# toposware/certificate-stark

Measured on NVIDIA B200. Metric: state_transition_prove_throughput, higher is better.
Workload: dtype u64 (f63 modular)

## Files before the change

certificate_stark_b200/csrc/prover.cu:

```cuda
#include "prover_ctx.cuh"

extern "C" {

csg_ctx *csg_create(int device) {
    int count = 0;
    if (cudaGetDeviceCount(&count) != cudaSuccess || device < 0 || device >= count) return nullptr;
    if (cudaSetDevice(device) != cudaSuccess) return nullptr;
    csg_ctx *ctx = new csg_ctx();
    ctx->device = device;
    if (cudaStreamCreateWithFlags(&ctx->st.s, cudaStreamNonBlocking) != cudaSuccess) { delete ctx; return nullptr; }
    return ctx;
}
void csg_destroy(csg_ctx *ctx) {
    if (!ctx) return;
    cudaSetDevice(ctx->device);
    cudaStreamSynchronize(ctx->st.s);
    cudaStream_t s = ctx->st.s;
    if (ctx->ev_a) { cudaEventDestroy(ctx->ev_a); cudaEventDestroy(ctx->ev_b); }
    for (auto e : ctx->cons_ev) if (e) cudaEventDestroy(e);
    for (auto e : ctx->chunk_ev) cudaEventDestroy(e);
    for (auto &e : ctx->comm_ev) { cudaEventDestroy(e.first); cudaEventDestroy(e.second); }
    if (ctx->ev_intt) { cudaEventDestroy(ctx->ev_intt); cudaEventDestroy(ctx->ev_gathered); }
    if (ctx->comm_stream.s) { cudaStreamSynchronize(ctx->comm_stream.s); cudaStreamDestroy(ctx->comm_stream.s); }
    ctx->comm.reset();
    if (ctx->copy_stream) cudaStreamDestroy(ctx->copy_stream);
    for (auto b : ctx->stage_buf) if (b) cudaFreeHost(b);
    for (auto e : ctx->stage_ev) if (e) cudaEventDestroy(e);
    if (ctx->h2d_a) { cudaEventDestroy(ctx->h2d_a); cudaEventDestroy(ctx->h2d_b); }
    many_delete(ctx->many);
    delete ctx;
    cudaStreamDestroy(s);
}
const char *csg_last_error(const csg_ctx *ctx) { return ctx ? ctx->err.c_str() : "no context (CUDA device unavailable)"; }
void csg_free(void *p) { free(p); }

int csg_set_air(csg_ctx *ctx, int air_id, size_t trace_len, const csg_options *opt, const uint64_t *pub, size_t npub) {
    return guarded(ctx, [&] { ctx->set_air(air_id, trace_len, opt, pub, npub); });
}
int csg_load_trace(csg_ctx *ctx, const uint64_t *trace, int repr) { return guarded(ctx, [&] { if (!trace) throw ArgError("null trace"); ctx->load_trace(trace, repr); }); }
int csg_reload_resident_trace(csg_ctx *ctx) { return guarded(ctx, [&] { ctx->reload_resident(); }); }
int csg_prove_loaded(csg_ctx *ctx, uint8_t **proof, size_t *proof_len) {
    return guarded(ctx, [&] { if (!proof || !proof_len) throw ArgError("null output"); ctx->prove_loaded(proof, proof_len); });
}
int csg_prove(csg_ctx *ctx, int air_id, const uint64_t *trace, int repr, size_t trace_len, const uint64_t *pub, size_t npub, const csg_options *opt,
              uint8_t **proof, size_t *proof_len) {
    return guarded(ctx, [&] {
        if (!trace || !proof || !proof_len) throw ArgError("null argument");
        csg_ctx::check_repr(repr);
        ctx->set_air(air_id, trace_len, opt, pub, npub);
        ctx->prove_loaded(proof, proof_len, trace, repr);
    });
}
int csg_prove_trace(csg_ctx *ctx, const uint64_t *trace, int repr, uint8_t **proof, size_t *proof_len) {
    return guarded(ctx, [&] {
        if (!trace || !proof || !proof_len) throw ArgError("null argument");
        csg_ctx::check_repr(repr);
        ctx->need(S_AIR, "csg_set_air must be called first");
        ctx->prove_loaded(proof, proof_len, trace, repr);
    });
}
int csg_prefetch_trace(csg_ctx *ctx, const uint64_t *trace, int repr) { return guarded(ctx, [&] { ctx->prefetch_trace(trace, repr); }); }
int csg_prove_prefetched(csg_ctx *ctx, const uint64_t *next_trace, int next_repr, uint8_t **proof, size_t *proof_len) {
    return guarded(ctx, [&] {
        if (!proof || !proof_len) throw ArgError("null argument");
        ctx->prove_prefetched(next_trace, next_repr, proof, proof_len);
    });
}
int csg_prove_columns(csg_ctx *ctx, int air_id, const uint64_t *const *columns, int repr, size_t trace_len, const uint64_t *pub, size_t npub,
                      const csg_options *opt, uint8_t **proof, size_t *proof_len) {
    return guarded(ctx, [&] {
        if (!columns || !proof || !proof_len) throw ArgError("null argument");
        csg_ctx::check_repr(repr);
        ctx->set_air(air_id, trace_len, opt, pub, npub);
        ctx->prove_loaded(proof, proof_len, nullptr, repr, columns);
    });
}
static int prove_many(csg_ctx *ctx, int air_id, size_t count, ManyTraces traces, int repr, size_t trace_len, const uint64_t *pubs, size_t npub,
                      const csg_options *opt, uint8_t **proofs, size_t *proof_lens) {
    if (proofs && proof_lens)
        for (size_t k = 0; k < count; k++) { proofs[k] = nullptr; proof_lens[k] = 0; }
    return guarded(ctx, [&] {
        if (ctx->comm && ctx->comm->world > 1) throw std::runtime_error("csg_prove_many does not run on a context attached to a group");
        if (!ctx->many) ctx->many = many_new();
        ctx->stage_timer.discard(); ctx->query_timer.discard();
        try { many_prove(ctx->many, ctx->st, air_id, count, traces, repr, trace_len, pubs, npub, opt, proofs, proof_lens, ctx->tm); }
        catch (const ManyArgError &e) { throw ArgError(e.what()); }
    });
}
int csg_prove_many(csg_ctx *ctx, int air_id, size_t count, const uint64_t *const *traces, int repr, size_t trace_len, const uint64_t *pubs, size_t npub,
                   const csg_options *opt, uint8_t **proofs, size_t *proof_lens) {
    return prove_many(ctx, air_id, count, ManyTraces{traces, nullptr}, repr, trace_len, pubs, npub, opt, proofs, proof_lens);
}
int csg_prove_many_device(csg_ctx *ctx, int air_id, size_t count, const uint64_t *traces_dev, int repr, size_t trace_len, const uint64_t *pubs,
                          size_t npub, const csg_options *opt, uint8_t **proofs, size_t *proof_lens) {
    return prove_many(ctx, air_id, count, ManyTraces{nullptr, traces_dev}, repr, trace_len, pubs, npub, opt, proofs, proof_lens);
}
void *csg_host_alloc(size_t bytes) {
    void *p = nullptr;
    if (!bytes || cudaHostAlloc(&p, bytes, cudaHostAllocPortable) != cudaSuccess) { cudaGetLastError(); return nullptr; }
    return p;
}
void csg_host_free(void *p) { if (p) cudaFreeHost(p); }
int csg_host_register(void *p, size_t bytes) {
    if (!p || !bytes) return CSG_ERR_ARG;
    if (cudaHostRegister(p, bytes, cudaHostRegisterDefault) != cudaSuccess) { cudaGetLastError(); return CSG_ERR_CUDA; }
    return CSG_OK;
}
int csg_host_unregister(void *p) {
    if (!p) return CSG_ERR_ARG;
    if (cudaHostUnregister(p) != cudaSuccess) { cudaGetLastError(); return CSG_ERR_CUDA; }
    return CSG_OK;
}
int csg_extend_and_commit_trace(csg_ctx *ctx, uint8_t root[32]) { return guarded(ctx, [&] { ctx->extend_and_commit_trace(root); }); }
int csg_eval_constraints(csg_ctx *ctx, const uint64_t *t_coeffs, const uint64_t *b_coeffs) {
    return guarded(ctx, [&] {
        ctx->need(S_AIR, "csg_set_air must be called first");
        if (ctx->d > 1) {
            std::vector<xe> t = mont_xvec(t_coeffs, 2 * ctx->air.num_constraints(), ctx->d), bb = mont_xvec(b_coeffs, 2 * ctx->air.assertions.size(), ctx->d);
            bb.push_back(x_zero());
            ctx->eval_constraints_x(t.data(), bb.data());
            return;
        }
        std::vector<fe> t = mont_vec(t_coeffs, 2 * ctx->air.num_constraints()), bb = mont_vec(b_coeffs, 2 * ctx->air.assertions.size());
        bb.push_back(0);
        ctx->eval_constraints(t.data(), bb.data());
    });
}
int csg_commit_composition(csg_ctx *ctx, uint8_t root[32]) { return guarded(ctx, [&] { ctx->commit_composition(root); }); }
int csg_ood_ext(csg_ctx *ctx, const uint64_t *z, uint64_t *frame_cur, uint64_t *frame_next, uint64_t *comp) {
    return guarded(ctx, [&] {
        if (!z || !frame_cur || !frame_next || !comp) throw ArgError("null argument");
        const int d = ctx->d;
        if (d == 1) { csg_ctx *c = ctx; c->ood(to_mont(z[0] % P)); for (size_t i = 0; i < c->air.width; i++) { frame_cur[i] = from_mont(c->ood_cur[i]); frame_next[i] = from_mont(c->ood_next[i]); }
                      for (size_t r = 0; r < c->ce; r++) comp[r] = from_mont(c->ood_comp[r]); return; }
        ctx->ood_x(mont_xvec(z, 1, d)[0]);
        for (size_t c = 0; c < ctx->air.width; c++)
            for (int j = 0; j < d; j++) { frame_cur[c * d + j] = from_mont(ctx->xood_cur[c].c[j]); frame_next[c * d + j] = from_mont(ctx->xood_next[c].c[j]); }
        for (size_t r = 0; r < ctx->ce; r++) for (int j = 0; j < d; j++) comp[r * d + j] = from_mont(ctx->xood_comp[r].c[j]);
    });
}
int csg_ood(csg_ctx *ctx, uint64_t z, uint64_t *frame_cur, uint64_t *frame_next, uint64_t *comp) {
    return guarded(ctx, [&] {
        if (ctx->d != 1) throw ArgError("with a field extension the out-of-domain point has several words: use csg_ood_ext");
        ctx->ood(to_mont(z % P));
        for (size_t c = 0; c < ctx->air.width; c++) { frame_cur[c] = from_mont(ctx->ood_cur[c]); frame_next[c] = from_mont(ctx->ood_next[c]); }
        for (size_t r = 0; r < ctx->ce; r++) comp[r] = from_mont(ctx->ood_comp[r]);
    });
}
int csg_deep(csg_ctx *ctx, const uint64_t *trace_ab, const uint64_t *comp_d, const uint64_t lambda_mu[2]) {
    return guarded(ctx, [&] {
        ctx->need(S_AIR, "csg_set_air must be called first");
        if (ctx->d > 1) {
            std::vector<xe> ab = mont_xvec(trace_ab, 2 * ctx->air.width, ctx->d), dd = mont_xvec(comp_d, ctx->ce, ctx->d), lm = mont_xvec(lambda_mu, 2, ctx->d);
            ctx->deep_x(ab.data(), dd.data(), lm[0], lm[1]);
            return;
        }
        std::vector<fe> ab = mont_vec(trace_ab, 2 * ctx->air.width), d = mont_vec(comp_d, ctx->ce);
        ctx->deep(ab.data(), d.data(), to_mont(lambda_mu[0] % P), to_mont(lambda_mu[1] % P));
    });
}
int csg_fri_commit_layer(csg_ctx *ctx, uint8_t root[32]) { return guarded(ctx, [&] { ctx->fri_commit_layer(root); }); }
int csg_fri_fold(csg_ctx *ctx, uint64_t alpha) {
    return guarded(ctx, [&] { if (ctx->d != 1) throw ArgError("with a field extension alpha has several words: use csg_fri_fold_ext"); ctx->fri_fold(to_mont(alpha % P)); });
}
int csg_fri_fold_ext(csg_ctx *ctx, const uint64_t *alpha) {
    return guarded(ctx, [&] { if (!alpha) throw ArgError("null argument"); ctx->fri_fold_x(mont_xvec(alpha, 1, ctx->d)[0]); });
}
int csg_fri_remainder(csg_ctx *ctx, uint64_t *out, size_t cap, size_t *len) {
    return guarded(ctx, [&] {
        ctx->need(S_DEEP, "the DEEP composition must be computed first");
        const FriLayer &L = *ctx->fri[ctx->nfri - 1];
        if (cap < L.m * ctx->d) throw ArgError("remainder buffer too small");
        std::vector<uint64_t> rem = ctx->remainder();
        memcpy(out, rem.data(), rem.size() * 8);
        *len = rem.size();
    });
}
static std::vector<size_t> checked_positions(const uint64_t *positions, size_t npos, size_t nleaves) {
    if (!positions || npos == 0 || npos > 255) throw ArgError("between 1 and 255 query positions");
    std::vector<size_t> pos(positions, positions + npos);
    std::vector<size_t> sorted(pos);
    std::sort(sorted.begin(), sorted.end());
    if (sorted.back() >= nleaves) throw ArgError("query position outside the evaluation domain");
    if (std::adjacent_find(sorted.begin(), sorted.end()) != sorted.end()) throw ArgError("query positions must be distinct");
    return pos;
}
static void copy_opening(const std::vector<uint64_t> &r, const std::vector<uint8_t> &p, uint64_t *rows, uint8_t *paths, size_t cap, size_t *paths_len) {
    if (!rows || !paths || !paths_len) throw ArgError("null output");
    if (p.size() > cap) throw ArgError("path buffer too small");
    memcpy(rows, r.data(), r.size() * 8);
    memcpy(paths, p.data(), p.size());
    *paths_len = p.size();
}
int csg_open_trace(csg_ctx *ctx, const uint64_t *positions, size_t npos, uint64_t *rows, uint8_t *paths, size_t cap, size_t *paths_len) {
    return guarded(ctx, [&] {
        ctx->need(S_COMMITTED, "the trace must be committed first");
        std::vector<size_t> pos = checked_positions(positions, npos, ctx->lde_n);
        const size_t w = ctx->air.width;
        copy_opening(ctx->open_rows(ctx->d_lde.p, (unsigned)w, (unsigned)ctx->b, w * ctx->n, ctx->n, pos, true), ctx->open_paths(ctx->d_tnodes, ctx->lde_n, pos, ctx->subtrees() ? &ctx->d_ttop : nullptr), rows, paths, cap, paths_len);
    });
}
int csg_open_composition(csg_ctx *ctx, const uint64_t *positions, size_t npos, uint64_t *rows, uint8_t *paths, size_t cap, size_t *paths_len) {
    return guarded(ctx, [&] {
        ctx->need(S_COMPOSED, "the composition polynomial must be committed first");
        std::vector<size_t> pos = checked_positions(positions, npos, ctx->lde_n);
        const size_t cw = ctx->ce * ctx->d;
        copy_opening(ctx->open_rows(ctx->d_clde.p, (unsigned)cw, (unsigned)ctx->b, cw * ctx->n, ctx->n, pos, true), ctx->open_paths(ctx->d_cnodes, ctx->lde_n, pos, ctx->subtrees() ? &ctx->d_ctop : nullptr), rows, paths, cap, paths_len);
    });
}
int csg_open_fri_layer(csg_ctx *ctx, size_t layer, const uint64_t *positions, size_t npos, uint64_t *rows, uint8_t *paths, size_t cap, size_t *paths_len) {
    return guarded(ctx, [&] {
        ctx->need(S_DEEP, "the DEEP composition must be computed first");
        if (layer >= ctx->nfri || !ctx->fri[layer]->committed) throw ArgError("no such committed FRI layer");
        const FriLayer &L = *ctx->fri[layer];
        std::vector<size_t> pos = checked_positions(positions, npos, L.m / 4);
        copy_opening(ctx->open_fri_rows(L, pos), ctx->open_paths(L.nodes, L.m / 4, pos), rows, paths, cap, paths_len);
    });
}

}
```

certificate_stark_b200/csrc/prover_ctx.cuh:

```cuda
#pragma once
#include <algorithm>
#include <chrono>
#include <cstdlib>
#include <cstring>
#include <memory>
#include <string>
#include <vector>

#include "../../include/csg.h"
#include "comm.cuh"
#include "commit.cuh"
#include "constraints.cuh"
#include "ext_stages.cuh"
#include "hash.cuh"
#include "host/air_desc.hpp"
#include "host/batch_plan.hpp"
#include "host/proof_common.hpp"
#include "host/transcript.hpp"
#include "many/many.cuh"
#include "ntt.cuh"
#include "stages.cuh"
#include "witness.cuh"


namespace csg {
using namespace f63;

namespace {

struct StateError : std::runtime_error { using std::runtime_error::runtime_error; };
struct ArgError : std::runtime_error { using std::runtime_error::runtime_error; };

struct FriLayer {
    DBuf<fe> owned;
    const fe *evals = nullptr;
    size_t m = 0;
    DBuf<uint32_t> nodes;
    bool committed = false;
};

enum Stage { S_NONE, S_AIR, S_TRACE, S_COMMITTED, S_EVALUATED, S_COMPOSED, S_OOD, S_DEEP };

class Timer {
  public:
    ~Timer() { for (auto &p : own_) { cudaEventDestroy(p.first); cudaEventDestroy(p.second); } }
    void start(Stream &st) {
        if (crowded()) flush();
        if (used_ == own_.size()) { cudaEvent_t a, b; CSG_CUDA(cudaEventCreate(&a)); CSG_CUDA(cudaEventCreate(&b)); own_.emplace_back(a, b); }
        l0_ = st.launches;
        CSG_CUDA(cudaEventRecord(own_[used_].first, st.s));
    }
    unsigned launches = 0;
    float stop(Stream &st) {
        launches = (unsigned)(st.launches - l0_);
        cudaEvent_t a = own_[used_].first, b = own_[used_].second;
        CSG_CUDA(cudaEventRecord(b, st.s)); CSG_CUDA(cudaEventSynchronize(b));
        float ms = 0; CSG_CUDA(cudaEventElapsedTime(&ms, a, b)); return ms;
    }
    void stop(Stream &st, float *dst, bool add = false) {
        launches = (unsigned)(st.launches - l0_);
        CSG_CUDA(cudaEventRecord(own_[used_].second, st.s));
        pending_.push_back({own_[used_].first, own_[used_].second, dst, add});
        used_++;
    }
    void span(cudaEvent_t a, cudaEvent_t b, float *dst, bool add = false) { pending_.push_back({a, b, dst, add}); }
    void zero(float *dst) { pending_.push_back({nullptr, nullptr, dst, false}); }
    bool crowded() const { return pending_.size() >= 256; }
    void discard() { pending_.clear(); used_ = 0; }
    void flush() {
        for (const Pending &q : pending_) {
            float ms = 0;
            if (q.a) { CSG_CUDA(cudaEventSynchronize(q.b)); CSG_CUDA(cudaEventElapsedTime(&ms, q.a, q.b)); }
            *q.dst = q.add ? *q.dst + ms : ms;
        }
        pending_.clear();
        used_ = 0;
    }
  private:
    struct Pending { cudaEvent_t a, b; float *dst; bool add; };
    std::vector<std::pair<cudaEvent_t, cudaEvent_t>> own_;
    std::vector<Pending> pending_;
    size_t used_ = 0;
    unsigned long long l0_ = 0;
};

}
}

using namespace csg;

static std::vector<size_t> trace_chunks(bool from_host, size_t c_lo, size_t c_hi) {
    std::vector<size_t> chunks;
    if (c_hi <= c_lo) return chunks;
    if (!from_host) { chunks.push_back(c_hi - c_lo); return chunks; }
    static const std::vector<size_t> sched = [] {
        std::vector<size_t> v;
        if (const char *e = getenv("CSG_H2D_CHUNKS"))
            for (const char *q = e; *q;) { char *end; const unsigned long x = strtoul(q, &end, 10); if (end == q) break; if (x) v.push_back(x); q = *end ? end + 1 : end; }
        if (v.empty()) v = {1, 3, 4, 8};
        return v;
    }();
    for (size_t c = c_lo, k = 0; c < c_hi; k++) { const size_t sz = std::min(sched[std::min(k, sched.size() - 1)], c_hi - c); chunks.push_back(sz); c += sz; }
    return chunks;
}

static bool shard_plan(size_t rank, size_t world, size_t b, size_t ce, size_t w, csg_shard_plan *out) {
    if (world < 1 || rank >= world || b < world || b % world || ce < 1 || ce > b || b % ce) return false;
    const size_t bl = b / world, k0 = rank * bl, cpr = (w + world - 1) / world;
    size_t kc0 = 0, cel = 0;
    for (size_t kc = 0; kc < ce; kc++) {
        const size_t k = kc * (b / ce);
        if (k >= k0 && k < k0 + bl) { if (!cel) kc0 = kc; cel++; }
    }
    const size_t c_lo = std::min(w, rank * cpr), c_hi = std::min(w, c_lo + cpr);
    *out = csg_shard_plan{(uint32_t)k0, (uint32_t)bl, (uint32_t)kc0, (uint32_t)cel, (uint32_t)c_lo, (uint32_t)(c_hi - c_lo), (uint32_t)cpr};
    return true;
}

struct csg_ctx {
    int device = 0;
    Stream st;
    std::string err;
    RootTable roots;
    NttScratch ntt;
    DBuf<fe> scratch, scratch2;
    Stage stage = S_NONE;

    AirDesc air;
    csg_options opt{};
    TransitionGroups tg;
    BoundaryGroups bg;
    size_t n = 0, b = 0, ce = 0, lde_n = 0;
    unsigned logn = 0;
    std::vector<fe> lde_shift, ce_shift;
    std::unique_ptr<Comm> comm;
    size_t G = 1, rank = 0, bl = 0, k0 = 0, cel = 0, kc0 = 0;
    DBuf<uint64_t> d_gather;
    DBuf<fe> d_xch;
    std::vector<std::pair<cudaEvent_t, cudaEvent_t>> comm_ev;
    size_t comm_used = 0;
    Stream comm_stream;
    cudaEvent_t ev_intt = nullptr, ev_gathered = nullptr;
    std::vector<cudaEvent_t> block_ev;

    DBuf<uint64_t> d_io, d_wit_in;
    DBuf<uint64_t> d_b_accounts, d_b_txw, d_b_sigs;
    DBuf<int> d_b_left, d_b_right, d_b_refs;
    DBuf<fe> d_b_hashes, d_b_defaults, d_b_gtable;
    unsigned b_defaults_depth = 0;
    bool b_gtable_built = false;
    size_t wit_resident_ntx = 0;
    unsigned wit_resident_depth = 0;
    DBuf<fe> d_wit_finals;
    std::vector<uint64_t> wit_packed;
    const csg_tx_batch *wit_packed_for = nullptr;
    DBuf<uint32_t> d_idx, d_dig;
    DBuf<fe> d_parts, d_polys, d_lde, d_comb, d_e, d_eg, d_cpolys, d_clde, d_abc, d_abc_lde, d_deep, d_ptab, d_apoly;
    DBuf<uint32_t> d_tnodes, d_cnodes;
    DBuf<uint32_t> d_ttop, d_ctop;
    bool subtrees() const { return G > 1 && n >= G; }
    uint32_t tree_ref(size_t idx) const {
        if (!subtrees()) return (uint32_t)idx;
        if (idx < 2 * G) return rank == 0 ? (0x80000000u | (uint32_t)idx) : 0xFFFFFFFFu;
        unsigned l = 0;
        while (((size_t)2 << l) <= idx) l++;
        const unsigned ls = l - ilog2(G);
        const size_t p = idx - ((size_t)1 << l);
        return (p >> ls) == rank ? (uint32_t)(((size_t)1 << ls) + (p & (((size_t)1 << ls) - 1))) : 0xFFFFFFFFu;
    }
    DBuf<ConsArgs> d_cargs;
    std::unique_ptr<ConsArgs> h_cargs;
    bool cargs_domain_ready = false;
    std::vector<std::unique_ptr<FriLayer>> fri;
    size_t nfri = 0;
    DBuf<uint64_t> d_rows;
    Timer stage_timer, query_timer;
    void flush_timers() { stage_timer.flush(); query_timer.flush(); }

    fe z = 0;
    std::vector<fe> ood_cur, ood_next, ood_comp;
    int d = 1;
    ExtConsts xk{};
    xe xz{};
    std::vector<xe> xood_cur, xood_next, xood_comp;
    DBuf<fe> d_pw;
    csg_timings tm{};
    cudaEvent_t ev_a = nullptr, ev_b = nullptr;
    cudaEvent_t cons_ev[6] = {nullptr, nullptr, nullptr, nullptr, nullptr, nullptr};
    bool split_low_degree = getenv("CSG_NO_SPLIT") == nullptr;
    size_t split_min_rows = getenv("CSG_SPLIT_MIN_ROWS") ? strtoull(getenv("CSG_SPLIT_MIN_ROWS"), nullptr, 10) : (size_t)1 << 14;
    cudaStream_t copy_stream = nullptr;
    std::vector<cudaEvent_t> chunk_ev;
    int trace_repr = CSG_REPR_CANONICAL;
    enum { STAGE_BUFS = 3 };
    uint64_t *stage_buf[STAGE_BUFS] = {nullptr, nullptr, nullptr};
    size_t stage_words = 0;
    cudaEvent_t stage_ev[STAGE_BUFS] = {nullptr, nullptr, nullptr};
    float h2d_ms_last = 0;
    cudaEvent_t h2d_a = nullptr, h2d_b = nullptr;
    CosetTables lde_tables;
    ManyProver *many = nullptr;

    void set_air(int air_id, size_t trace_len, const csg_options *o, const uint64_t *pub, size_t npub) {
        try { check_options(o); } catch (const std::invalid_argument &e) { throw ArgError(e.what()); }
        const bool same_shape = stage >= S_AIR && air.id == air_id && n == trace_len && memcmp(&opt, o, sizeof opt) == 0 &&
                                G == (comm ? (size_t)comm->world : 1) && rank == (comm ? (size_t)comm->rank : 0);
        bool same_periodic = same_shape;
        {
            AirDesc fresh;
            try { fresh = make_air(air_id, trace_len, pub, npub); } catch (const std::invalid_argument &e) { throw ArgError(e.what()); }
            same_periodic = same_periodic && fresh.periodic.size() == air.periodic.size();
            for (size_t c = 0; same_periodic && c < fresh.periodic.size(); c++) same_periodic = fresh.periodic[c].values == air.periodic[c].values;
            if (!(same_shape && same_periodic)) {
                stage = S_NONE;
                if (next_pending) { CSG_CUDA(cudaStreamSynchronize(copy_stream)); next_pending = false; }
            }
            air = std::move(fresh);
        }
        if (same_shape && same_periodic) {
            tg = transition_groups(air);
            bg = boundary_groups(air);
            cargs_domain_ready = false;
            nfri = 0;
            stage = S_AIR;
            return;
        }
        opt = *o;
        d = (int)o->field_extension;
        if (d > 1) xk = ext_consts();
        n = trace_len; logn = ilog2(n); b = o->blowup_factor; ce = air.ce_blowup(); lde_n = n * b;
        if (ce > b) throw ArgError("blowup factor is smaller than the constraint evaluation blowup of this AIR");
        G = comm ? (size_t)comm->world : 1; rank = comm ? (size_t)comm->rank : 0;
        csg_shard_plan plan;
        if (!shard_plan(rank, G, b, ce, air.width, &plan)) throw ArgError("the number of ranks of a sharded proof must divide the blowup factor");
        bl = plan.num_cosets; k0 = plan.first_coset;
        if (logn > 22) throw ArgError("trace length above 2^22 is not supported");
        try { check_remainder(lde_n, *o); } catch (const std::invalid_argument &e) { throw ArgError(e.what()); }
        if (air.num_constraints() > (size_t)CONS_MAX_CONSTRAINTS || air.periodic.size() > (size_t)CONS_MAX_PERIODIC ||
            air.assertions.size() > (size_t)CONS_MAX_ASSERTIONS)
            throw ArgError("AIR exceeds the compiled table sizes");
        tg = transition_groups(air);
        bg = boundary_groups(air);
        if (tg.adj.size() > (size_t)CONS_MAX_GROUPS || bg.groups.size() > (size_t)CONS_MAX_BGROUPS) throw ArgError("too many constraint groups");
        roots.build(logn, st);
        const fe offset = to_mont(GENERATOR), w_lde = root_of_unity(ilog2(lde_n));
        std::vector<fe> all_shift(b);
        fe acc = offset;
        for (size_t k = 0; k < b; k++) { all_shift[k] = acc; acc = mul(acc, w_lde); }
        lde_shift.assign(all_shift.begin() + k0, all_shift.begin() + k0 + bl);
        ce_shift.clear();
        kc0 = plan.first_ce_coset; cel = plan.num_ce_cosets;
        for (size_t kc = kc0; kc < kc0 + cel; kc++) ce_shift.push_back(all_shift[kc * (b / ce)]);
        build_periodic_tables();
        lde_tables.build(lde_shift.data(), bl, logn, st);
        nfri = 0;
        stage = S_AIR;
    }

    void build_periodic_tables() {
        h_cargs.reset(new ConsArgs());
        cargs_domain_ready = false;
        ConsArgs &A = *h_cargs;
        memset(&A, 0, sizeof A);
        const size_t np = air.periodic.size();
        A.nperiodic = (unsigned)np;
        size_t total = 0;
        for (size_t c = 0; c < np; c++) {
            const size_t P = air.periodic[c].values.size();
            if (P == 0 || (P & (P - 1)) || P > n) throw ArgError("periodic column length must be a power of two dividing the trace length");
            A.poff[c] = (unsigned)total; A.pmask[c] = (unsigned)(P - 1);
            total += P;
        }
        A.ptab_coset_stride = total;
        d_ptab.reserve((total ? total : 1) * (cel ? cel : 1));
        std::vector<bool> done(np, false);
        DBuf<fe> vals, coef;
        for (size_t c0 = 0; c0 < np; c0++) {
            if (done[c0]) continue;
            const size_t P = air.periodic[c0].values.size();
            size_t c1 = c0;
            while (c1 < np && air.periodic[c1].values.size() == P) { done[c1] = true; c1++; }
            const size_t nc = c1 - c0;
            std::vector<fe> host(nc * P);
            for (size_t c = c0; c < c1; c++) memcpy(&host[(c - c0) * P], air.periodic[c].values.data(), P * sizeof(fe));
            vals.reserve(nc * P); coef.reserve(nc * P);
            CSG_CUDA(cudaMemcpyAsync(vals.p, host.data(), nc * P * sizeof(fe), cudaMemcpyHostToDevice, st.s));
            intt_columns(roots, ntt, vals.p, P, coef.p, P, nc, ilog2(P), st);
            std::vector<fe> shifts(cel);
            for (size_t kc = 0; kc < cel; kc++) shifts[kc] = f63::pow(ce_shift[kc], n / P);
            if (cel) coset_ntt_columns(roots, ntt, coef.p, P, d_ptab.p + A.poff[c0], P, total, nc, ilog2(P), shifts.data(), cel, st);
            CSG_CUDA(cudaStreamSynchronize(st.s));
        }
    }

    static void check_repr(int repr) { if (repr != CSG_REPR_CANONICAL && repr != CSG_REPR_MONTGOMERY) throw ArgError("repr must be CSG_REPR_CANONICAL or CSG_REPR_MONTGOMERY"); }
    static bool is_pageable(const void *p) {
        cudaPointerAttributes a{};
        if (cudaPointerGetAttributes(&a, p) != cudaSuccess) { cudaGetLastError(); return true; }
        return a.type == cudaMemoryTypeUnregistered;
    }
    void load_trace(const uint64_t *trace, int repr) {
        need(S_AIR, "csg_set_air must be called first");
        check_repr(repr);
        trace_repr = repr;
        const size_t count = (size_t)air.width * n;
        Timer &t = stage_timer;
        t.start(st);
        d_io.reserve(count);
        CSG_CUDA(cudaMemcpyAsync(d_io.p, trace, count * sizeof(uint64_t), cudaMemcpyHostToDevice, st.s));
        tm.h2d = t.stop(st);
        nfri = 0;
        stage = S_TRACE;
    }
    DBuf<uint64_t> d_next;
    cudaEvent_t next_a = nullptr, next_b = nullptr;
    bool next_pending = false;
    int next_repr = CSG_REPR_CANONICAL;
    void prefetch_trace(const uint64_t *trace, int repr) {
        need(S_AIR, "csg_set_air must be called first");
        check_repr(repr);
        if (!trace) throw ArgError("null trace");
        if (next_pending) throw StateError("a prefetched trace is already waiting: csg_prove_prefetched proves it");
        csg_shard_plan plan;
        shard_plan(rank, G, b, ce, air.width, &plan);
        d_next.reserve((size_t)air.width * n);
        if (!copy_stream) CSG_CUDA(cudaStreamCreateWithFlags(&copy_stream, cudaStreamNonBlocking));
        if (!next_a) { CSG_CUDA(cudaEventCreate(&next_a)); CSG_CUDA(cudaEventCreate(&next_b)); }
        CSG_CUDA(cudaEventRecord(next_a, copy_stream));
        if (plan.num_columns)
            CSG_CUDA(cudaMemcpyAsync(d_next.p + (size_t)plan.first_column * n, trace + (size_t)plan.first_column * n,
                                     (size_t)plan.num_columns * n * sizeof(uint64_t), cudaMemcpyHostToDevice, copy_stream));
        CSG_CUDA(cudaEventRecord(next_b, copy_stream));
        next_repr = repr;
        next_pending = true;
    }
    void prove_prefetched(const uint64_t *next_trace, int next_trace_repr, uint8_t **proof, size_t *proof_len) {
        if (!next_pending) throw StateError("csg_prefetch_trace must be called first");
        CSG_CUDA(cudaEventSynchronize(next_b));
        CSG_CUDA(cudaEventElapsedTime(&tm.h2d, next_a, next_b));
        std::swap(d_io.p, d_next.p); std::swap(d_io.n, d_next.n);
        trace_repr = next_repr;
        next_pending = false;
        nfri = 0;
        stage = S_TRACE;
        if (next_trace) prefetch_trace(next_trace, next_trace_repr);
        prove_loaded(proof, proof_len);
    }
    void reload_resident() {
        need(S_TRACE, "no trace has been loaded");
        nfri = 0;
        stage = S_TRACE;
        tm.h2d = 0;
    }

    void need(Stage s, const char *msg) const { if (stage < s) throw StateError(msg); }
    void download_root(const DBuf<uint32_t> &nodes, uint8_t root[32]) {
        CSG_CUDA(cudaMemcpyAsync(root, nodes.p + 8, 32, cudaMemcpyDeviceToHost, st.s));
        CSG_CUDA(cudaStreamSynchronize(st.s));
    }
    void all_to_all(const void *send, void *recv, size_t bytes) {
        comm_events();
        CSG_CUDA(cudaEventRecord(comm_ev[comm_used].first, st.s));
        comm->all_to_all(send, recv, bytes, st);
        CSG_CUDA(cudaEventRecord(comm_ev[comm_used++].second, st.s));
    }

    void extend_and_commit_trace(uint8_t root[32], const uint64_t *host = nullptr, int host_repr = CSG_REPR_CANONICAL, const uint64_t *const *host_cols = nullptr) {
        std::vector<const uint64_t *> colptr;
        if (host || host_cols) {
            check_repr(host_repr); trace_repr = host_repr;
            colptr.resize(air.width);
            for (size_t c = 0; c < air.width; c++) {
                colptr[c] = host_cols ? host_cols[c] : host + c * n;
                if (!colptr[c]) throw ArgError("null trace column");
            }
            if (!host) host = colptr[0];
        }
        if (!host) need(S_TRACE, "csg_load_trace must be called first");
        else need(S_AIR, "csg_set_air must be called first");
        const size_t w = air.width;
        csg_shard_plan plan;
        shard_plan(rank, G, b, ce, w, &plan);
        const size_t cpr = plan.columns_per_rank, c_lo = plan.first_column, c_hi = c_lo + plan.num_columns, wpad = cpr * G;
        const std::vector<size_t> chunks = trace_chunks(host != nullptr, c_lo, c_hi);
        size_t CHUNK = 1;
        for (size_t s : chunks) CHUNK = std::max(CHUNK, s);
        Timer &t = stage_timer;
        t.start(st);
        d_io.reserve(w * n); d_polys.reserve(wpad * n); scratch.reserve(wpad * n); d_lde.reserve(w * n * bl);
        bool any_pageable = false;
        if (host) for (size_t c = c_lo; c < c_hi && !any_pageable; c++) any_pageable = is_pageable(colptr[c]);
        const bool staged = host && any_pageable;
        if (host) {
            if (!copy_stream) CSG_CUDA(cudaStreamCreateWithFlags(&copy_stream, cudaStreamNonBlocking));
            while (chunk_ev.size() < chunks.size() + 1) { cudaEvent_t e; CSG_CUDA(cudaEventCreateWithFlags(&e, cudaEventDisableTiming)); chunk_ev.push_back(e); }
            if (!h2d_a) { CSG_CUDA(cudaEventCreate(&h2d_a)); CSG_CUDA(cudaEventCreate(&h2d_b)); }
            if (staged && stage_words < CHUNK * n) {
                for (auto &b : stage_buf) { if (b) cudaFreeHost(b); b = nullptr; }
                for (auto &b : stage_buf) CSG_CUDA(cudaHostAlloc((void **)&b, CHUNK * n * sizeof(uint64_t), cudaHostAllocDefault));
                stage_words = CHUNK * n;
                for (auto &e : stage_ev) if (!e) CSG_CUDA(cudaEventCreateWithFlags(&e, cudaEventDisableTiming));
            }
            CSG_CUDA(cudaEventRecord(chunk_ev[0], st.s));
            CSG_CUDA(cudaStreamWaitEvent(copy_stream, chunk_ev[0], 0));
            CSG_CUDA(cudaEventRecord(h2d_a, copy_stream));
        }
        for (size_t c0 = c_lo, k = 0; k < chunks.size() && c0 < c_hi; c0 += chunks[k], k++) {
            const size_t nc = std::min(chunks[k], c_hi - c0);
            if (host) {
                bool contiguous = true;
                for (size_t j = 1; j < nc; j++) contiguous = contiguous && colptr[c0 + j] == colptr[c0] + j * n;
                const uint64_t *src = colptr[c0];
                if (staged) {
                    uint64_t *buf = stage_buf[k % STAGE_BUFS];
                    if (k >= STAGE_BUFS) CSG_CUDA(cudaEventSynchronize(stage_ev[k % STAGE_BUFS]));
                    const size_t SL = (size_t)1 << 17, per_col = (n + SL - 1) / SL;
                    const long long nsl = (long long)(per_col * nc);
#pragma omp parallel for schedule(static)
                    for (long long sl = 0; sl < nsl; sl++) {
                        const size_t j = (size_t)sl / per_col, o = ((size_t)sl % per_col) * SL;
                        memcpy(buf + j * n + o, colptr[c0 + j] + o, std::min(SL, n - o) * sizeof(uint64_t));
                    }
                    src = buf; contiguous = true;
                }
                if (contiguous) CSG_CUDA(cudaMemcpyAsync(d_io.p + c0 * n, src, nc * n * sizeof(uint64_t), cudaMemcpyHostToDevice, copy_stream));
                else for (size_t j = 0; j < nc; j++)
                    CSG_CUDA(cudaMemcpyAsync(d_io.p + (c0 + j) * n, colptr[c0 + j], n * sizeof(uint64_t), cudaMemcpyHostToDevice, copy_stream));
                if (staged) CSG_CUDA(cudaEventRecord(stage_ev[k % STAGE_BUFS], copy_stream));
                CSG_CUDA(cudaEventRecord(chunk_ev[k], copy_stream));
                if (c0 + nc >= c_hi) CSG_CUDA(cudaEventRecord(h2d_b, copy_stream));
                CSG_CUDA(cudaStreamWaitEvent(st.s, chunk_ev[k], 0));
            }
            intt_columns(roots, ntt, d_io.p + c0 * n, n, scratch.p + c0 * n, n, nc, logn, st, trace_repr == CSG_REPR_MONTGOMERY ? 0 : R2, true);
            if (G == 1) coset_ntt_columns(roots, ntt, scratch.p + c0 * n, n, d_lde.p + c0 * n, n, w * n, nc, logn, lde_tables, st);
        }
        if (G > 1) {
            static const bool one_gather = getenv("CSG_COEF_BLOCKWISE") == nullptr;
            if (!comm_stream.s) CSG_CUDA(cudaStreamCreateWithFlags(&comm_stream.s, cudaStreamNonBlocking));
            if (!ev_intt) { CSG_CUDA(cudaEventCreateWithFlags(&ev_intt, cudaEventDisableTiming)); CSG_CUDA(cudaEventCreateWithFlags(&ev_gathered, cudaEventDisableTiming)); }
            while (block_ev.size() < G) { cudaEvent_t e; CSG_CUDA(cudaEventCreateWithFlags(&e, cudaEventDisableTiming)); block_ev.push_back(e); }
            CSG_CUDA(cudaEventRecord(ev_intt, st.s));
            if (c_hi > c_lo) coset_ntt_columns(roots, ntt, scratch.p + c_lo * n, n, d_lde.p + c_lo * n, n, w * n, c_hi - c_lo, logn, lde_tables, st);
            CSG_CUDA(cudaStreamWaitEvent(comm_stream.s, ev_intt, 0));
            if (one_gather) {
                gather(scratch.p, cpr * n * sizeof(fe), &comm_stream);
                CSG_CUDA(cudaEventRecord(ev_gathered, comm_stream.s));
                CSG_CUDA(cudaStreamWaitEvent(st.s, ev_gathered, 0));
                if (c_lo > 0) coset_ntt_columns(roots, ntt, scratch.p, n, d_lde.p, n, w * n, c_lo, logn, lde_tables, st);
                if (c_hi < w) coset_ntt_columns(roots, ntt, scratch.p + c_hi * n, n, d_lde.p + c_hi * n, n, w * n, w - c_hi, logn, lde_tables, st);
            } else {
                for (unsigned q = 0; q < G; q++) {
                    const size_t q_lo = std::min((size_t)q * cpr, w), q_hi = std::min(q_lo + cpr, w);
                    bcast(scratch.p + (size_t)q * cpr * n, cpr * n * sizeof(fe), (int)q, &comm_stream);
                    if (q == rank || q_hi == q_lo) continue;
                    CSG_CUDA(cudaEventRecord(block_ev[q], comm_stream.s));
                    CSG_CUDA(cudaStreamWaitEvent(st.s, block_ev[q], 0));
                    coset_ntt_columns(roots, ntt, scratch.p + q_lo * n, n, d_lde.p + q_lo * n, n, w * n, q_hi - q_lo, logn, lde_tables, st);
                }
                CSG_CUDA(cudaEventRecord(ev_gathered, comm_stream.s));
                CSG_CUDA(cudaStreamWaitEvent(st.s, ev_gathered, 0));
            }
        }
        std::swap(d_polys.p, scratch.p); std::swap(d_polys.n, scratch.n);
        t.stop(st, &tm.lde); tm.stage_launches[0] = t.launches;
        if (host) {
            nfri = 0;
            t.zero(&tm.h2d);
            if (c_hi > c_lo) t.span(h2d_a, h2d_b, &tm.h2d);
        }
        t.start(st);
        commit_rows(d_lde.p, (unsigned)w, w * n, d_tnodes, d_ttop);
        download_root(subtrees() ? d_ttop : d_tnodes, root);
        t.stop(st, &tm.commit_trace); tm.stage_launches[1] = t.launches;
        stage = S_COMMITTED;
    }

    void comm_events() {
        if (comm_ev.size() == comm_used) {
            cudaEvent_t a, e;
            CSG_CUDA(cudaEventCreate(&a)); CSG_CUDA(cudaEventCreate(&e));
            comm_ev.emplace_back(a, e);
        }
    }
    void gather(void *buf, size_t bytes, Stream *on = nullptr) {
        Stream &cs = on ? *on : st;
        comm_events();
        CSG_CUDA(cudaEventRecord(comm_ev[comm_used].first, cs.s));
        comm->all_gather(buf, bytes, cs);
        CSG_CUDA(cudaEventRecord(comm_ev[comm_used++].second, cs.s));
    }
    void bcast(void *buf, size_t bytes, int root, Stream *on = nullptr) {
        Stream &cs = on ? *on : st;
        comm_events();
        CSG_CUDA(cudaEventRecord(comm_ev[comm_used].first, cs.s));
        comm->broadcast(buf, bytes, root, cs);
        CSG_CUDA(cudaEventRecord(comm_ev[comm_used++].second, cs.s));
    }
    void reduce_rows(uint64_t *buf, size_t count) {
        comm_events();
        CSG_CUDA(cudaEventRecord(comm_ev[comm_used].first, st.s));
        comm->all_reduce_sum_u64(buf, count, st);
        CSG_CUDA(cudaEventRecord(comm_ev[comm_used++].second, st.s));
    }
    float comm_ms() {
        float total = 0;
        for (size_t i = 0; i < comm_used; i++) {
            float ms = 0;
            CSG_CUDA(cudaEventSynchronize(comm_ev[i].second));
            CSG_CUDA(cudaEventElapsedTime(&ms, comm_ev[i].first, comm_ev[i].second));
            total += ms;
        }
        return total;
    }
    DBuf<fe> d_ood_xch;
    std::vector<fe> gather_column_values(const std::vector<fe> &mine, size_t per_col, size_t ncols) {
        csg_shard_plan plan;
        shard_plan(rank, G, b, ce, ncols, &plan);
        const size_t cpr = plan.columns_per_rank, slice = cpr * per_col;
        d_ood_xch.reserve(std::max<size_t>(slice * G, 64));
        std::vector<fe> padded(slice, 0);
        std::copy(mine.begin(), mine.end(), padded.begin());
        CSG_CUDA(cudaMemcpyAsync(d_ood_xch.p + rank * slice, padded.data(), slice * sizeof(fe), cudaMemcpyHostToDevice, st.s));
        gather(d_ood_xch.p, slice * sizeof(fe));
        std::vector<fe> all(slice * G);
        CSG_CUDA(cudaMemcpyAsync(all.data(), d_ood_xch.p, all.size() * sizeof(fe), cudaMemcpyDeviceToHost, st.s));
        CSG_CUDA(cudaStreamSynchronize(st.s));
        all.resize(ncols * per_col);
        return all;
    }
    void commit_rows(const fe *data, unsigned width, size_t coset_stride, DBuf<uint32_t> &nodes, DBuf<uint32_t> &top) {
        const int hf = (int)opt.hash_fn;
        if (G == 1) {
            nodes.reserve(16 * lde_n);
            hash_rows(data, width, n, (unsigned)b, coset_stride, n, hf, nodes.p + 8 * lde_n, st);
            merkle_build(nodes.p, lde_n, hf, st);
            return;
        }
        if (!subtrees()) {
            nodes.reserve(16 * lde_n);
            d_gather.reserve(4 * lde_n);
            hash_rows(data, width, n, (unsigned)bl, coset_stride, n, hf, (uint32_t *)d_gather.p + 8 * rank * bl * n, st);
            gather(d_gather.p, bl * n * 32);
            interleave_slices(d_gather.p, (uint64_t *)(nodes.p + 8 * lde_n), n, (unsigned)bl, (unsigned)G, 4, st);
            merkle_build(nodes.p, lde_n, hf, st);
            return;
        }
        const size_t nl = lde_n / G, chunk = (n / G) * bl * 32;
        nodes.reserve(16 * nl); top.reserve(16 * G);
        d_gather.reserve(8 * bl * n);
        uint64_t *send = d_gather.p, *recv = d_gather.p + 4 * bl * n;
        hash_rows(data, width, n, (unsigned)bl, coset_stride, n, hf, (uint32_t *)send, st);
        all_to_all(send, recv, chunk);
        interleave_slices(recv, (uint64_t *)(nodes.p + 8 * nl), n / G, (unsigned)bl, (unsigned)G, 4, st);
        merkle_build(nodes.p, nl, hf, st);
        CSG_CUDA(cudaMemcpyAsync(top.p + 8 * (G + rank), nodes.p + 8, 32, cudaMemcpyDeviceToDevice, st.s));
        gather(top.p + 8 * G, 32);
        merkle_build(top.p, G, hf, st);
    }

    void eval_constraints(const fe *t_ab, const fe *b_ab, int plane = 0, bool all_components = false) {
        need(S_COMMITTED, "the trace must be committed first");
        Timer &t = stage_timer;
        t.start(st);
        ConsArgs &A = *h_cargs;
        A.ext_degree = all_components ? (unsigned)d : 1;
        for (size_t i = 0; i < air.num_constraints(); i++) { A.alpha[i] = t_ab[2 * i]; A.beta[i] = t_ab[2 * i + 1]; A.group[i] = tg.group_of[i]; }
        A.nconstraints = (unsigned)air.num_constraints(); A.ngroups = (unsigned)tg.adj.size();
        fill_rescue_tables(air.id, A);
        for (size_t i = 0; i < air.assertions.size(); i++) { A.a_alpha[i] = b_ab[2 * i]; A.a_beta[i] = b_ab[2 * i + 1]; }
        host_mark("  cons: coefficient tables");
        if (!cargs_domain_ready) {
            const fe g = root_of_unity(logn);
            A.logn = logn; A.ncosets = (unsigned)cel; A.col_stride = n; A.width = air.width;
            A.g_last = f63::pow(g, n - 1);
            for (size_t gi = 0; gi < tg.adj.size(); gi++) A.adj_mod[gi] = tg.adj[gi] % n;
            A.nbgroups = (unsigned)bg.groups.size(); A.nassertions = (unsigned)air.assertions.size();
            for (size_t gi = 0; gi < bg.groups.size(); gi++) {
                A.b_adj_mod[gi] = bg.groups[gi].adj % n; A.b_steps[gi] = bg.groups[gi].num_steps; A.b_offset[gi] = bg.groups[gi].offset;
            }
            for (size_t kc = 0; kc < cel; kc++) {
                const fe s = ce_shift[kc];
                A.lde_coset_stride[kc] = (unsigned long long)((kc0 + kc) * (b / ce) - k0) * air.width * n;
                A.shift[kc] = s;
                A.zinv[kc] = inv(sub(f63::pow(s, n), ONE));
                for (size_t gi = 0; gi < tg.adj.size(); gi++) A.shift_adj[kc][gi] = f63::pow(s, tg.adj[gi]);
                for (size_t gi = 0; gi < bg.groups.size(); gi++) {
                    A.b_shift_adj[kc][gi] = f63::pow(s, bg.groups[gi].adj);
                    A.b_shift_steps[kc][gi] = f63::pow(s, bg.groups[gi].num_steps);
                }
            }
            std::vector<fe> polys;
            const fe g_inv = inv(g);
            for (size_t i = 0; i < air.assertions.size(); i++) {
                const Assertion &s = air.assertions[i];
                A.a_col[i] = s.column; A.a_group[i] = bg.group_of[i];
                A.a_value[i] = s.values[0]; A.a_poly_len[i] = (unsigned)s.values.size(); A.a_poly_off[i] = polys.size();
                A.a_xoff[i] = s.first_step ? f63::pow(g_inv, s.first_step) : ONE;
                if (s.values.size() > 1) {
                    std::vector<fe> c = interpolate_host(s.values);
                    polys.insert(polys.end(), c.begin(), c.end());
                }
            }
            d_apoly.reserve(polys.size() ? polys.size() : 1);
            if (!polys.empty()) {
                CSG_CUDA(cudaMemcpyAsync(d_apoly.p, polys.data(), polys.size() * sizeof(fe), cudaMemcpyHostToDevice, st.s));
                CSG_CUDA(cudaStreamSynchronize(st.s));
            }
            cargs_domain_ready = true;
        }
        d_cargs.reserve(1);
        CSG_CUDA(cudaMemcpyAsync(d_cargs.p, &A, sizeof A, cudaMemcpyHostToDevice, st.s));
        const size_t comb_plane = (cel ? cel : 1) * n;
        d_comb.reserve(comb_plane * d);
        d_parts.reserve(constraint_scratch_elements(air.id, n, cel ? cel : 1) * (all_components ? d : 1));
        host_mark("  cons: args upload, scratch");
        if (!cons_ev[0]) for (auto &e : cons_ev) CSG_CUDA(cudaEventCreate(&e));
        const bool split = split_low_degree && n >= split_min_rows && (G == 1 || (ce == b && bl % 2 == 0));
        SplitExchange xch{(unsigned)G, (unsigned)rank, [](void *self, void *buf, size_t bytes) { static_cast<csg_ctx *>(self)->gather(buf, bytes); }, this, nullptr, 0};
        if (split && G > 1) {
            d_xch.reserve((size_t)16 * d * (ce / 2) * n);
            xch.buf = d_xch.p; xch.buf_elems = d_xch.n;
        }
        const SplitExchange *px = split && G > 1 ? &xch : nullptr;
        if (cel && all_components) csg::eval_constraints_ext(air.id, d_cargs.p, A, d_lde.p, roots.W.p, d_ptab.p, d_apoly.p, d_parts.p, d_comb.p, st, cons_ev,
                                                             split ? &roots : nullptr, split ? &ntt : nullptr, px);
        else if (cel) csg::eval_constraints(air.id, d_cargs.p, A, d_lde.p, roots.W.p, d_ptab.p, d_apoly.p, d_parts.p, d_comb.p + plane * comb_plane, st, cons_ev,
                                            split ? &roots : nullptr, split ? &ntt : nullptr, px);
        else for (auto &e : cons_ev) CSG_CUDA(cudaEventRecord(e, st.s));
        t.stop(st, &tm.constraints, plane != 0);
        tm.stage_launches[2] = plane ? tm.stage_launches[2] + t.launches : t.launches;
        float *parts_ms[4] = {&tm.cons_rescue, &tm.cons_ecc_banks, &tm.cons_ecc_final, &tm.cons_rest};
        for (int k = 0; k < 4; k++) t.span(cons_ev[k], cons_ev[k + 1], parts_ms[k], plane != 0);
        t.span(cons_ev[1], cons_ev[5], &tm.cons_ecc_low, plane != 0);
        if (d > 1 && !all_components) t.flush();
        if (plane + 1 == d || all_components) stage = S_EVALUATED;
    }
    void eval_constraints_x(const xe *t_ab, const xe *b_ab) {
        const size_t nc = air.num_constraints(), na = air.assertions.size();
        std::vector<fe> tj(2 * nc), bj(2 * na + 2);
        if (getenv("CSG_EXT_PASSES")) {
            for (int j = 0; j < d; j++) {
                for (size_t i = 0; i < 2 * nc; i++) tj[i] = t_ab[i].c[j];
                for (size_t i = 0; i < 2 * na; i++) bj[i] = b_ab[i].c[j];
                eval_constraints(tj.data(), bj.data(), j);
            }
            return;
        }
        ConsArgs &A = *h_cargs;
        for (int j = 1; j < d; j++) {
            for (size_t i = 0; i < nc; i++) { A.alpha_x[j - 1][i] = t_ab[2 * i].c[j]; A.beta_x[j - 1][i] = t_ab[2 * i + 1].c[j]; }
            for (size_t i = 0; i < na; i++) { A.a_alpha_x[j - 1][i] = b_ab[2 * i].c[j]; A.a_beta_x[j - 1][i] = b_ab[2 * i + 1].c[j]; }
        }
        for (size_t i = 0; i < 2 * nc; i++) tj[i] = t_ab[i].c[0];
        for (size_t i = 0; i < 2 * na; i++) bj[i] = b_ab[i].c[0];
        eval_constraints(tj.data(), bj.data(), 0, true);
    }
    void commit_composition(uint8_t root[32]) {
        need(S_EVALUATED, "constraints must be evaluated first");
        Timer &t = stage_timer;
        t.start(st);
        std::vector<fe> sinv(cel);
        for (size_t kc = 0; kc < cel; kc++) sinv[kc] = inv(ce_shift[kc]);
        d_e.reserve(ce * n); d_cpolys.reserve(ce * d * n);
        std::vector<fe> mat(ce * ce);
        const fe off_n_inv = inv(f63::pow(to_mont(GENERATOR), n)), ce_inv = inv(to_mont(ce)), w_ce_inv = inv(root_of_unity(ilog2(ce)));
        for (size_t tt = 0; tt < ce; tt++)
            for (size_t k = 0; k < ce; k++)
                mat[tt * ce + k] = mul(mul(f63::pow(off_n_inv, tt), ce_inv), f63::pow(w_ce_inv, (k * tt) % ce));
        for (int j = 0; j < d; j++) {
        const fe *comb = d_comb.p + (size_t)j * (cel ? cel : 1) * n;
        const fe *e_all = d_e.p;
        if (G == 1) coset_intt_columns(roots, ntt, comb, n, d_e.p, n, logn, sinv.data(), ce, st);
        else {
            const size_t slot = cel ? cel : 1;
            d_eg.reserve(G * slot * n);
            if (cel) coset_intt_columns(roots, ntt, comb, n, d_eg.p + rank * slot * n, n, logn, sinv.data(), cel, st);
            gather(d_eg.p, slot * n * sizeof(fe));
            if (G <= ce) e_all = d_eg.p;
            else for (size_t kc = 0; kc < ce; kc++)
                CSG_CUDA(cudaMemcpyAsync(d_e.p + kc * n, d_eg.p + kc * (G / ce) * n, n * sizeof(fe), cudaMemcpyDeviceToDevice, st.s));
        }
        composition_columns(e_all, d_cpolys.p + (size_t)j * n, n, (unsigned)ce, mat.data(), st, (size_t)d * n);
        }
        const size_t cw = ce * d;
        d_clde.reserve(cw * n * bl);
        coset_ntt_columns(roots, ntt, d_cpolys.p, n, d_clde.p, n, cw * n, cw, logn, lde_shift.data(), bl, st);
        commit_rows(d_clde.p, (unsigned)cw, cw * n, d_cnodes, d_ctop);
        download_root(subtrees() ? d_ctop : d_cnodes, root);
        t.stop(st, &tm.composition); tm.stage_launches[3] = t.launches;
        stage = S_COMPOSED;
    }

    void ood(fe z_) {
        need(S_COMPOSED, "the composition polynomial must be committed first");
        Timer &t = stage_timer;
        t.start(st);
        z = z_;
        const size_t w = air.width;
        const fe pts[2] = {z, mul(z, root_of_unity(logn))};
        std::vector<fe> vals(2 * w);
        if (G == 1) eval_polys_at(d_polys.p, n, w, n, pts, 2, vals.data(), scratch2, st);
        else {
            csg_shard_plan plan;
            shard_plan(rank, G, b, ce, w, &plan);
            const size_t c_lo = plan.first_column, nc = plan.num_columns;
            std::vector<fe> blk(2 * nc), mine(2 * nc);
            if (nc) eval_polys_at(d_polys.p + c_lo * n, n, nc, n, pts, 2, blk.data(), scratch2, st);
            for (size_t c = 0; c < nc; c++) { mine[2 * c] = blk[c]; mine[2 * c + 1] = blk[nc + c]; }
            const std::vector<fe> all = gather_column_values(mine, 2, w);
            for (size_t c = 0; c < w; c++) { vals[c] = all[2 * c]; vals[w + c] = all[2 * c + 1]; }
        }
        ood_cur.assign(vals.begin(), vals.begin() + w);
        ood_next.assign(vals.begin() + w, vals.end());
        const fe zm = f63::pow(z, ce);
        ood_comp.resize(ce);
        eval_polys_at(d_cpolys.p, n, ce, n, &zm, 1, ood_comp.data(), scratch2, st);
        t.stop(st, &tm.ood_deep); tm.stage_launches[4] = t.launches;
        stage = S_OOD;
    }
    void deep(const fe *trace_ab, const fe *comp_d, fe lambda, fe mu) {
        need(S_OOD, "the out-of-domain frame must be computed first");
        Timer &t = stage_timer;
        t.start(st);
        const size_t w = air.width;
        std::vector<fe> coef(2 * w);
        DeepArgs a{};
        a.z = z; a.zg = mul(z, root_of_unity(logn)); a.zm = f63::pow(z, ce);
        for (size_t c = 0; c < w; c++) {
            coef[c] = trace_ab[2 * c]; coef[w + c] = trace_ab[2 * c + 1];
            a.az = add(a.az, mul(coef[c], ood_cur[c]));
            a.bzg = add(a.bzg, mul(coef[w + c], ood_next[c]));
        }
        for (size_t r = 0; r < ce; r++) a.czm = add(a.czm, mul(comp_d[r], ood_comp[r]));
        a.lambda = lambda; a.mu = mu; a.ncosets = (unsigned)bl;
        for (size_t k = 0; k < bl; k++) a.shift[k] = lde_shift[k];
        d_abc.reserve(3 * n); d_abc_lde.reserve(3 * n * bl); d_deep.reserve(lde_n);
        combine_polys(d_polys.p, n, w, n, coef.data(), 2, d_abc.p, n, scratch2, st);
        combine_polys(d_cpolys.p, n, ce, n, comp_d, 1, d_abc.p + 2 * n, n, scratch, st);
        coset_ntt_columns(roots, ntt, d_abc.p, n, d_abc_lde.p, n, 3 * n, 3, logn, lde_shift.data(), bl, st);
        if (G == 1) deep_quotients(d_abc_lde.p, roots.W.p, n, a, d_deep.p, st);
        else {
            d_gather.reserve(lde_n);
            deep_quotients(d_abc_lde.p, roots.W.p, n, a, (fe *)d_gather.p + rank * bl * n, st);
            gather(d_gather.p, bl * n * sizeof(fe));
            interleave_slices(d_gather.p, (uint64_t *)d_deep.p, n, (unsigned)bl, (unsigned)G, 1, st);
        }
        if (fri.empty()) fri.emplace_back(new FriLayer());
        nfri = 1;
        fri[0]->evals = d_deep.p; fri[0]->m = lde_n; fri[0]->committed = false;
        t.stop(st, &tm.ood_deep, true); tm.stage_launches[4] += t.launches;
        t.zero(&tm.fri); tm.stage_launches[5] = 0;
        stage = S_DEEP;
    }

    void ood_x(const xe &z_) {
        need(S_COMPOSED, "the composition polynomial must be committed first");
        Timer &t = stage_timer;
        t.start(st);
        xz = z_;
        const size_t w = air.width, cw = ce * d;
        const xe pts[2] = {xz, x_scale(xz, root_of_unity(logn))};
        d_pw.reserve(2 * (size_t)d * n);
        ext_power_table(d, pts, 2, n, d_pw.p, st);
        std::vector<fe> vals(w * 2 * d);
        if (G == 1) dot_columns(d_polys.p, n, w, n, d_pw.p, 2 * d, vals.data(), scratch2, st);
        else {
            csg_shard_plan plan;
            shard_plan(rank, G, b, ce, w, &plan);
            const size_t c_lo = plan.first_column, nc = plan.num_columns;
            std::vector<fe> mine(nc * 2 * d);
            if (nc) dot_columns(d_polys.p + c_lo * n, n, nc, n, d_pw.p, 2 * d, mine.data(), scratch2, st);
            vals = gather_column_values(mine, 2 * (size_t)d, w);
        }
        xood_cur.assign(w, x_zero()); xood_next.assign(w, x_zero());
// ... 375 lines not shown
```

Measured before the change: 17380.

## Overlap per-coset LDE with BLAKE3 leaf hashing on a high-priority stream

For large single-device traces hashed with BLAKE3, the trace LDE is now computed one coset at a time using per-coset tables. Each coset's leaf rows are hashed on a separate high-priority stream as soon as that coset is ready, and the leaf digests are then interleaved into Merkle node order before the tree is built. This is meant to hide row-hashing time behind the remaining coset NTTs instead of hashing after the full LDE. The cost is extra per-coset table memory, extra events and streams, and a dependence on the interleave layout matching the commit_rows ordering.

```diff
diff --git a/certificate_stark_b200/csrc/prover.cu b/certificate_stark_b200/csrc/prover.cu
--- a/certificate_stark_b200/csrc/prover.cu
+++ b/certificate_stark_b200/csrc/prover.cu
@@ -27,6 +27,8 @@
     for (auto b : ctx->stage_buf) if (b) cudaFreeHost(b);
     for (auto e : ctx->stage_ev) if (e) cudaEventDestroy(e);
     if (ctx->h2d_a) { cudaEventDestroy(ctx->h2d_a); cudaEventDestroy(ctx->h2d_b); }
+    for (auto e : ctx->hash_ev) cudaEventDestroy(e);
+    if (ctx->hash_stream) { cudaStreamSynchronize(ctx->hash_stream); cudaStreamDestroy(ctx->hash_stream); }
     many_delete(ctx->many);
     delete ctx;
     cudaStreamDestroy(s);
diff --git a/certificate_stark_b200/csrc/prover_ctx.cuh b/certificate_stark_b200/csrc/prover_ctx.cuh
--- a/certificate_stark_b200/csrc/prover_ctx.cuh
+++ b/certificate_stark_b200/csrc/prover_ctx.cuh
@@ -199,6 +199,10 @@
     float h2d_ms_last = 0;
     cudaEvent_t h2d_a = nullptr, h2d_b = nullptr;
     CosetTables lde_tables;
+    static constexpr size_t STREAMED_MIN_ROWS = (size_t)1 << 19;
+    std::vector<std::unique_ptr<CosetTables>> coset_tables;
+    cudaStream_t hash_stream = nullptr;
+    std::vector<cudaEvent_t> hash_ev;
     ManyProver *many = nullptr;
 
     void set_air(int air_id, size_t trace_len, const csg_options *o, const uint64_t *pub, size_t npub) {
@@ -253,6 +257,12 @@
         for (size_t kc = kc0; kc < kc0 + cel; kc++) ce_shift.push_back(all_shift[kc * (b / ce)]);
         build_periodic_tables();
         lde_tables.build(lde_shift.data(), bl, logn, st);
+        coset_tables.clear();
+        if (G == 1 && n >= STREAMED_MIN_ROWS)
+            for (size_t k = 0; k < bl; k++) {
+                coset_tables.emplace_back(new CosetTables());
+                coset_tables.back()->build(&lde_shift[k], 1, logn, st);
+            }
         nfri = 0;
         stage = S_AIR;
     }
@@ -382,6 +392,9 @@
         csg_shard_plan plan;
         shard_plan(rank, G, b, ce, w, &plan);
         const size_t cpr = plan.columns_per_rank, c_lo = plan.first_column, c_hi = c_lo + plan.num_columns, wpad = cpr * G;
+        static const bool streamed_on = !(getenv("CSG_STREAMED_COMMIT") && strcmp(getenv("CSG_STREAMED_COMMIT"), "0") == 0);
+        const bool streamed = streamed_on && !host && G == 1 && (int)opt.hash_fn == hashes::BLAKE3_256 && n >= STREAMED_MIN_ROWS &&
+                              coset_tables.size() == bl;
         const std::vector<size_t> chunks = trace_chunks(host != nullptr, c_lo, c_hi);
         size_t CHUNK = 1;
         for (size_t s : chunks) CHUNK = std::max(CHUNK, s);
@@ -432,7 +445,28 @@
                 CSG_CUDA(cudaStreamWaitEvent(st.s, chunk_ev[k], 0));
             }
             intt_columns(roots, ntt, d_io.p + c0 * n, n, scratch.p + c0 * n, n, nc, logn, st, trace_repr == CSG_REPR_MONTGOMERY ? 0 : R2, true);
-            if (G == 1) coset_ntt_columns(roots, ntt, scratch.p + c0 * n, n, d_lde.p + c0 * n, n, w * n, nc, logn, lde_tables, st);
+            if (G == 1 && !streamed) coset_ntt_columns(roots, ntt, scratch.p + c0 * n, n, d_lde.p + c0 * n, n, w * n, nc, logn, lde_tables, st);
+        }
+        if (streamed) {
+            d_tnodes.reserve(16 * lde_n);
+            d_gather.reserve(4 * lde_n);
+            if (!hash_stream) {
+                int least = 0, greatest = 0;
+                CSG_CUDA(cudaDeviceGetStreamPriorityRange(&least, &greatest));
+                CSG_CUDA(cudaStreamCreateWithPriority(&hash_stream, cudaStreamNonBlocking, greatest));
+            }
+            while (hash_ev.size() < bl + 1) { cudaEvent_t e; CSG_CUDA(cudaEventCreateWithFlags(&e, cudaEventDisableTiming)); hash_ev.push_back(e); }
+            Stream hs{hash_stream, 0};
+            for (size_t k = 0; k < bl; k++) {
+                coset_ntt_columns(roots, ntt, scratch.p, n, d_lde.p + k * w * n, n, w * n, w, logn, *coset_tables[k], st);
+                CSG_CUDA(cudaEventRecord(hash_ev[k], st.s));
+                CSG_CUDA(cudaStreamWaitEvent(hash_stream, hash_ev[k], 0));
+                hash_rows(d_lde.p + k * w * n, (unsigned)w, n, 1, w * n, n, (int)opt.hash_fn, (uint32_t *)d_gather.p + 8 * k * n, hs);
+            }
+            interleave_slices(d_gather.p, (uint64_t *)(d_tnodes.p + 8 * lde_n), n, 1, (unsigned)bl, 4, hs);
+            st.launches += hs.launches;
+            CSG_CUDA(cudaEventRecord(hash_ev[bl], hash_stream));
+            CSG_CUDA(cudaStreamWaitEvent(st.s, hash_ev[bl], 0));
         }
         if (G > 1) {
             static const bool one_gather = getenv("CSG_COEF_BLOCKWISE") == nullptr;
@@ -469,7 +503,8 @@
             if (c_hi > c_lo) t.span(h2d_a, h2d_b, &tm.h2d);
         }
         t.start(st);
-        commit_rows(d_lde.p, (unsigned)w, w * n, d_tnodes, d_ttop);
+        if (streamed) merkle_build(d_tnodes.p, lde_n, (int)opt.hash_fn, st);
+        else commit_rows(d_lde.p, (unsigned)w, w * n, d_tnodes, d_ttop);
         download_root(subtrees() ? d_ttop : d_tnodes, root);
         t.stop(st, &tm.commit_trace); tm.stage_launches[1] = t.launches;
         stage = S_COMMITTED;
```

Result: slower. 17190 (median of 6 runs) (-1.1%).
